# stdstu12/YUME

Measured on AMD Instinct MI355X. Metric: denoise-steps/sec (Yume-5B 720P, 33-frame latent), higher is better.
Workload: dtype bf16; 1 GPU; Yume-5B-720P random-init, 33-frame 704x1280 clip (latent 48x13x44x80, FramePack lfz=8, L=9460), ODE Euler steps of a 50-step shift-7 schedule, no CFG, one chain per GPU; num_layers=30, parallelism=dp1 (independent chains, replicated weights)

## Files before the change

yume_amd/csrc/gemm_w4.hpp:

```cpp
#pragma once
#include "gemm_core.hpp"
#include "trace.hpp"

namespace gemm_w4 {
using namespace gemm_core;

constexpr int NTHR_W4 = 256;
constexpr int OPER_BYTES = 256 * 128;
constexpr int BUF_BYTES = 2 * OPER_BYTES;
constexpr int LDS_W4 = 2 * BUF_BYTES;

#define W4_AG8(n) "a" #n "0", "a" #n "1", "a" #n "2", "a" #n "3", "a" #n "4", "a" #n "5", "a" #n "6", "a" #n "7", "a" #n "8", "a" #n "9"
#define W4_AGPRS "a0", "a1", "a2", "a3", "a4", "a5", "a6", "a7", "a8", "a9", W4_AG8(1), W4_AG8(2), W4_AG8(3), W4_AG8(4), W4_AG8(5), W4_AG8(6), \
    W4_AG8(7), W4_AG8(8), W4_AG8(9), W4_AG8(10), W4_AG8(11), W4_AG8(12), W4_AG8(13), W4_AG8(14), W4_AG8(15), W4_AG8(16), W4_AG8(17), W4_AG8(18), \
    W4_AG8(19), W4_AG8(20), W4_AG8(21), W4_AG8(22), W4_AG8(23), W4_AG8(24), "a250", "a251", "a252", "a253", "a254", "a255"

#define W4_MFMA2(T0, X0, Y0, T1, X1, Y1)                                                                                                         \
    asm volatile("v_mfma_f32_16x16x32_bf16 a[%c4:%c5], %0, %1, a[%c4:%c5]\n\tv_mfma_f32_16x16x32_bf16 a[%c6:%c7], %2, %3, a[%c6:%c7]"             \
                 ::"v"(X0), "v"(Y0), "v"(X1), "v"(Y1), "n"((T0) * 4), "n"((T0) * 4 + 3), "n"((T1) * 4), "n"((T1) * 4 + 3) : "memory", W4_AGPRS)
#define W4_MFMA2_DMA(T0, X0, Y0, T1, X1, Y1, voff, sbase, lbase, loff)                                                                            \
    asm volatile("s_add_u32 m0, %10, %11\n\tv_mfma_f32_16x16x32_bf16 a[%c4:%c5], %0, %1, a[%c4:%c5]\n\tglobal_load_lds_dwordx4 %8, %9\n\t"         \
                 "v_mfma_f32_16x16x32_bf16 a[%c6:%c7], %2, %3, a[%c6:%c7]"                                                                       \
                 ::"v"(X0), "v"(Y0), "v"(X1), "v"(Y1), "n"((T0) * 4), "n"((T0) * 4 + 3), "n"((T1) * 4), "n"((T1) * 4 + 3), "v"(voff), "s"(sbase),   \
                 "s"(lbase), "n"(loff) : "memory", "scc", W4_AGPRS)
#define W4_MFMA2_DMAB(T0, X0, Y0, T1, X1, Y1, voff, srd, soff, lbase, loff)                                                                           \
    asm volatile("s_add_u32 m0, %11, %12\n\tv_mfma_f32_16x16x32_bf16 a[%c4:%c5], %0, %1, a[%c4:%c5]\n\tbuffer_load_dwordx4 %8, %9, %10 offen lds\n\t"  \
                 "v_mfma_f32_16x16x32_bf16 a[%c6:%c7], %2, %3, a[%c6:%c7]"                                                                           \
                 ::"v"(X0), "v"(Y0), "v"(X1), "v"(Y1), "n"((T0) * 4), "n"((T0) * 4 + 3), "n"((T1) * 4), "n"((T1) * 4 + 3), "v"(voff), "s"(srd),         \
                 "s"(soff), "s"(lbase), "n"(loff) : "memory", "scc", W4_AGPRS)
#define W4_DMAB(voff, srd, soff, lbase, loff) \
    asm volatile("s_add_u32 m0, %3, %4\n\ts_nop 0\n\tbuffer_load_dwordx4 %0, %1, %2 offen lds" ::"v"(voff), "s"(srd), "s"(soff), "s"(lbase), "n"(loff) : "memory", "scc")
#define W4_DMA(voff, sbase, lbase, loff) \
    asm volatile("s_add_u32 m0, %2, %3\n\ts_nop 0\n\tglobal_load_lds_dwordx4 %0, %1" ::"v"(voff), "s"(sbase), "s"(lbase), "n"(loff) : "memory", "scc")

template <int R>
__device__ __forceinline__ f32x4 acc_tile() {
    f32x4 v;
    asm volatile("v_accvgpr_read_b32 %0, a[%c4]\n\tv_accvgpr_read_b32 %1, a[%c5]\n\tv_accvgpr_read_b32 %2, a[%c6]\n\tv_accvgpr_read_b32 %3, a[%c7]"
                 : "=v"(v[0]), "=v"(v[1]), "=v"(v[2]), "=v"(v[3]) : "n"(R * 4), "n"(R * 4 + 1), "n"(R * 4 + 2), "n"(R * 4 + 3) : W4_AGPRS);
    return v;
}
template <int R>
__device__ __forceinline__ void acc_tile_add(f32x4 d) {
    f32x4 v = acc_tile<R>();
    v += d;
    asm volatile("v_accvgpr_write_b32 a[%c4], %0\n\tv_accvgpr_write_b32 a[%c5], %1\n\tv_accvgpr_write_b32 a[%c6], %2\n\tv_accvgpr_write_b32 a[%c7], %3"
                 ::"v"(v[0]), "v"(v[1]), "v"(v[2]), "v"(v[3]), "n"(R * 4), "n"(R * 4 + 1), "n"(R * 4 + 2), "n"(R * 4 + 3) : W4_AGPRS);
}
template <int R0, int N>
__device__ __forceinline__ void acc_zero() {
    if constexpr (N > 0) {
        asm volatile("v_accvgpr_write_b32 a[%c0], 0\n\tv_accvgpr_write_b32 a[%c1], 0\n\tv_accvgpr_write_b32 a[%c2], 0\n\tv_accvgpr_write_b32 a[%c3], 0"
                     ::"n"(R0), "n"(R0 + 1), "n"(R0 + 2), "n"(R0 + 3) : W4_AGPRS);
        acc_zero<R0 + 4, N - 4>();
    }
}
template <int I0, int N, typename F>
__device__ __forceinline__ void static_for(F&& f) {
    if constexpr (N > 0) {
        f(std::integral_constant<int, I0>{});
        static_for<I0 + 1, N - 1>(f);
    }
}

struct Ctx {
    char* smem;
    bf16x8_t fa[2][8], fb[2][8];
    unsigned ra1, rb1, ra0n, rb0n;
    unsigned va[8], vb[8];
    const char* pa;
    const char* pb;
    unsigned lcur;
    i32x4 srd;
    unsigned soff, tapmask;
    unsigned mask[8];
    unsigned par[8];
    unsigned uh[2], uw[2];
};

__device__ __forceinline__ bf16x8_t w4_frag(const Ctx& c, unsigned off) { return *reinterpret_cast<const bf16x8_t*>(c.smem + off); }

#define W4_PIECE_LOFF(q) (((q) >> 3) * OPER_BYTES + ((q) & 7) * 4096)

#define W4_X(g) (SWAP ? c.fb[(g) >> 6][(g) & 7] : c.fa[(g) >> 6][((g) & 63) >> 3])
#define W4_Y(g) (SWAP ? c.fa[(g) >> 6][((g) & 63) >> 3] : c.fb[(g) >> 6][(g) & 7])
#define W4_PAIR(g) W4_MFMA2((g) & 63, W4_X(g), W4_Y(g), ((g) + 1) & 63, W4_X((g) + 1), W4_Y((g) + 1))
#define W4_PAIR_DMA(g, voff, sbase, loff) \
    W4_MFMA2_DMA((g) & 63, W4_X(g), W4_Y(g), ((g) + 1) & 63, W4_X((g) + 1), W4_Y((g) + 1), voff, sbase, c.lcur, loff)
#define W4_PAIR_DMAB(g, voff, loff) \
    W4_MFMA2_DMAB((g) & 63, W4_X(g), W4_Y(g), ((g) + 1) & 63, W4_X((g) + 1), W4_Y((g) + 1), voff, c.srd, c.soff, c.lcur, loff)

#ifndef W4_PLAN
#define W4_PLAN 1
#endif
#ifndef W4_ABLATE
#define W4_ABLATE 0
#endif
#ifndef W4_BAR_B
#define W4_BAR_B 35
#endif
#ifndef W4_BAR_A
#define W4_BAR_A 17
#endif
#ifndef W4_DMA0
#define W4_DMA0 (W4_BAR_A + 2)
#endif
constexpr int P_BAR_A = W4_BAR_A;
constexpr int P_BAR_B = W4_BAR_B;
constexpr int dma_pos(int q) { return W4_PLAN == 0 ? W4_DMA0 + q : W4_DMA0 + (q * (63 - W4_DMA0)) / 15; }
constexpr int piece_at(int pos) {
    for (int q = 0; q < 16; ++q)
        if (dma_pos(q) == pos) return q;
    return -1;
}
constexpr int pieces_before_bar_b() {
    int k = 0;
    for (int q = 0; q < 16; ++q) k += dma_pos(q) <= P_BAR_B ? 1 : 0;
    return k;
}
constexpr int P_F0_FIRST = P_BAR_B + 2;
static_assert(P_F0_FIRST + 16 <= 64 && dma_pos(15) <= 63 && 15 < P_BAR_A && dma_pos(0) > P_BAR_A, "the plan must fit the 64 slots");

template <int CONV>
__device__ __forceinline__ unsigned w4_conv_voff(const Ctx& c, int q) {
    unsigned v = c.va[q];
    if constexpr (CONV == 2) v += ((c.par[q] & 1u) ? c.uh[1] : c.uh[0]) + ((c.par[q] & 2u) ? c.uw[1] : c.uw[0]);
    return (c.mask[q] & c.tapmask) ? v : 0xffffffffu;
}

template <int g, bool DMA, bool SWAP, int CONV>
__device__ __forceinline__ void w4_gaps(Ctx& c) {
    if constexpr (g < 128) {
        {
            constexpr int k = g >> 1, pos = k;
            constexpr int q = (DMA && !(W4_ABLATE & 1)) ? piece_at(pos) : -1;
            if constexpr (q >= 0 && q < 8) {
                if constexpr (CONV != 0) W4_PAIR_DMAB(g, w4_conv_voff<CONV>(c, q & 7), W4_PIECE_LOFF(q & 15));
                else W4_PAIR_DMA(g, c.va[q & 7], c.pa, W4_PIECE_LOFF(q & 15));
            } else if constexpr (q >= 8) W4_PAIR_DMA(g, c.vb[q & 7], c.pb, W4_PIECE_LOFF(q & 15));
            else W4_PAIR(g);
            if constexpr (pos >= 0 && pos < 16 && !(W4_ABLATE & 2)) {
                if constexpr (pos < 8) c.fb[1][pos & 7] = w4_frag(c, c.rb1 + (pos & 7) * 2048);
                else c.fa[1][pos & 7] = w4_frag(c, c.ra1 + (pos & 7) * 2048);
            }
            if constexpr (k == P_BAR_A) {
                if constexpr ((W4_ABLATE & 20) == 20) asm volatile("" ::: "memory");
                else if constexpr (W4_ABLATE & 16) asm volatile("s_barrier" ::: "memory");
                else if constexpr (W4_ABLATE & 4) asm volatile("s_waitcnt lgkmcnt(0)" ::: "memory");
                else asm volatile("s_waitcnt lgkmcnt(0)\n\ts_barrier" ::: "memory");
            }
            if constexpr (k == P_BAR_B) {
                constexpr int keep = (DMA && !(W4_ABLATE & 1)) ? pieces_before_bar_b() : 0;
                if constexpr ((W4_ABLATE & 12) == 12) asm volatile("" ::: "memory");
                else if constexpr (W4_ABLATE & 8) asm volatile("s_barrier" ::: "memory");
                else if constexpr (W4_ABLATE & 4) asm volatile("s_waitcnt vmcnt(%c0)" ::"n"(keep) : "memory");
                else asm volatile("s_waitcnt vmcnt(%c0)\n\ts_barrier" ::"n"(keep) : "memory");
            }
            if constexpr (pos >= P_F0_FIRST && pos < P_F0_FIRST + 16 && !(W4_ABLATE & 2)) {
                constexpr int r = pos - P_F0_FIRST;
                if constexpr (r < 8) c.fb[0][r & 7] = w4_frag(c, c.rb0n + (r & 7) * 2048);
                else c.fa[0][r & 7] = w4_frag(c, c.ra0n + (r & 7) * 2048);
            }
            w4_gaps<g + 2, DMA, SWAP, CONV>(c);
        }
    }
}
template <int q, int CONV>
__device__ __forceinline__ void w4_stage_all(Ctx& c) {
    if constexpr (q < 16) {
        if constexpr (q < 8) {
            if constexpr (CONV != 0) W4_DMAB(w4_conv_voff<CONV>(c, q & 7), c.srd, c.soff, c.lcur, W4_PIECE_LOFF(q));
            else W4_DMA(c.va[q & 7], c.pa, c.lcur, W4_PIECE_LOFF(q));
        } else W4_DMA(c.vb[q & 7], c.pb, c.lcur, W4_PIECE_LOFF(q));
        w4_stage_all<q + 1, CONV>(c);
    }
}

template <int EPI>
__device__ __forceinline__ f32x4 w4_act(f32x4 v) {
    if (EPI == YUME_EPI_BF16_GELU) {
        const f32x2_t lo = gelu_tanh2(f32x2_t{v[0], v[1]}), hi = gelu_tanh2(f32x2_t{v[2], v[3]});
        v = f32x4{lo[0], lo[1], hi[0], hi[1]};
    }
    if (EPI == YUME_EPI_BF16_GELU_ERF) {
#pragma unroll
        for (int q = 0; q < 4; ++q) v[q] = 0.5f * v[q] * (1.0f + erff(v[q] * 0.7071067811865476f));
    }
    return v;
}

__device__ __forceinline__ void w4_store_image(char* smem, unsigned short* dst, int64_t ld, int row0, int rows_valid, int col0, int cols_valid) {
    const int lane = threadIdx.x & 63;
    const int wave = __builtin_amdgcn_readfirstlane(threadIdx.x >> 6);
    const int l31 = lane & 31, rh = lane >> 5;
    if (cols_valid == 256) {
        const unsigned lrow = (unsigned)((wave * 64 + rh) * 512), lch = (unsigned)((l31 ^ rh) << 4);
        char* o = reinterpret_cast<char*>(dst + col0 + l31 * 8) + (int64_t)(row0 + wave * 64 + rh) * ld * 2;
        const int64_t step = ld * 4;
        const int rleft = rows_valid - wave * 64 - rh;
        auto rows = [&](auto pred) {
            constexpr bool PRED = decltype(pred)::value;
#pragma unroll
            for (int g = 0; g < 4; ++g) {
                u32x4 d[8];
#pragma unroll
                for (int u = 0; u < 8; ++u) {
                    const int it = g * 8 + u;
                    d[u] = *reinterpret_cast<const u32x4*>(smem + lrow + it * 1024 + (lch ^ (unsigned)(32 * (it & 15))));
                }
#pragma unroll
                for (int u = 0; u < 8; ++u) {
                    const int it = g * 8 + u;
                    if (!PRED || 2 * it < rleft) *reinterpret_cast<u32x4*>(o + it * step) = d[u];
                }
            }
        };
        if (rows_valid == 256) rows(std::false_type{});
        else rows(std::true_type{});
        return;
    }
    unsigned short* out = dst + col0 + l31 * 8;
    const int col_left = cols_valid - l31 * 8;
#pragma unroll 2
    for (int it = 0; it < 32; ++it) {
        const int r = wave * 64 + it * 2 + rh;
        const u32x4 d = *reinterpret_cast<const u32x4*>(smem + r * 512 + (((l31 ^ r) & 31) << 4));
        if (r < rows_valid && col_left > 0) {
            unsigned short* o = out + (int64_t)(row0 + r) * ld;
            if (col_left >= 8) {
                *reinterpret_cast<u32x4*>(o) = d;
            } else {
#pragma unroll
                for (int q = 0; q < 7; ++q)
                    if (q < col_left) o[q] = (unsigned short)(d[q >> 1] >> (16 * (q & 1)));
            }
        }
    }
}

struct ImageOff { unsigned e[8], o[8]; };
__device__ __forceinline__ ImageOff w4_image_offsets(int rsel, int csel, int l15, int l4) {
    ImageOff r;
    const unsigned base = (unsigned)((rsel * 128 + l15) * 512 + (l4 & 1) * 8), ux = (unsigned)(((l4 >> 1) ^ l15) << 4);
#pragma unroll
    for (int b = 0; b < 8; ++b) {
        const unsigned ob = (unsigned)(32 * b) ^ ux;
        r.e[b] = base + 256u * (unsigned)csel + ob;
        r.o[b] = base + 256u * (unsigned)(csel ^ 1) + ob;
    }
    return r;
}

template <int EPI, bool SWAP>
__device__ __forceinline__ void w4_epilogue(const Problem& p, const Epilogue& e, int m0, int n0, char* smem) {
    const int lane = threadIdx.x & 63;
    const int wave = __builtin_amdgcn_readfirstlane(threadIdx.x >> 6);
    const int wr = wave >> 1, wc = wave & 1;
    const int l15 = lane & 15, l4 = lane >> 4;
    constexpr bool BF16_OUT = EPI == YUME_EPI_BF16 || EPI == YUME_EPI_BF16_GELU || EPI == YUME_EPI_BF16_GELU_ERF || EPI == YUME_EPI_BF16_SPLITT ||
                              EPI == EPI_BF16_ADD || EPI == EPI_BF16_TSPLIT;
    if constexpr (!SWAP) {
        float bn[8];
#pragma unroll
        for (int j = 0; j < 8; ++j) bn[j] = e.bias ? e.bias[min(n0 + wc * 128 + 16 * j + l15, p.N - 1)] : 0.f;
        const ImageOff io = w4_image_offsets(wc, wr, l15, l4);
        asm volatile("s_waitcnt lgkmcnt(0)\n\ts_barrier" ::: "memory");
        static_for<0, 64>([&](auto tt) {
            constexpr int T = decltype(tt)::value, i = T >> 3, j = T & 7;
            const f32x4 v = acc_tile<T>();
            u32x2 o;
            o[0] = pack_bf16x2(v[0] + bn[j], v[1] + bn[j]);
            o[1] = pack_bf16x2(v[2] + bn[j], v[3] + bn[j]);
            *reinterpret_cast<u32x2*>(smem + ((j & 1) ? io.o[i] : io.e[i]) + j * 8192) = o;
        });
        asm volatile("s_waitcnt lgkmcnt(0)\n\ts_barrier" ::: "memory");
        w4_store_image(smem, e.outT + (int64_t)(n0 - e.n_split) * e.ldt, e.ldt, 0, min(256, p.N - n0), m0, min(256, p.M - m0));
        return;
    } else {
        if (BF16_OUT && !p.epi_direct && (e.ldo % 8) == 0) {
            f32x4 b[8];
            if (n0 + 256 <= p.N) {
#pragma unroll
                for (int j = 0; j < 8; ++j)
                    b[j] = e.bias ? *reinterpret_cast<const f32x4*>(e.bias + n0 + wc * 128 + 16 * j + 4 * l4) : f32x4{0.f, 0.f, 0.f, 0.f};
            } else {
#pragma unroll
                for (int j = 0; j < 8; ++j) {
                    const int n = n0 + wc * 128 + 16 * j + 4 * l4;
                    b[j] = (e.bias && n + 3 < p.N) ? *reinterpret_cast<const f32x4*>(e.bias + n) : f32x4{0.f, 0.f, 0.f, 0.f};
                }
            }
            const ImageOff io = w4_image_offsets(wr, wc, l15, l4);
            asm volatile("s_waitcnt lgkmcnt(0)\n\ts_barrier" ::: "memory");
            TRACE_STAMP(3);
            static_for<0, 8>([&](auto ii) {
                constexpr int i = decltype(ii)::value;
                u32x2 a2[8];
                if constexpr (EPI == EPI_BF16_ADD) {
                    const int r = wr * 128 + 16 * i + l15;
                    const int nl = n0 + wc * 128 + 4 * l4;
                    const unsigned short* ap = e.add + (int64_t)min(m0 + r, p.M - 1) * e.ldadd + nl;
#pragma unroll
                    for (int j = 0; j < 8; ++j)
                        a2[j] = nl + 16 * j + 3 < p.N ? *reinterpret_cast<const u32x2*>(ap + 16 * j) : u32x2{0u, 0u};
                }
                static_for<0, 8>([&](auto jj) {
                    constexpr int j = decltype(jj)::value;
                    f32x4 v = w4_act<EPI>(acc_tile<i * 8 + j>() + b[j]);
                    if constexpr (EPI == EPI_BF16_ADD) {
                        v[0] += bf16_to_f32((unsigned short)(a2[j][0] & 0xffffu));
                        v[1] += bf16_to_f32((unsigned short)(a2[j][0] >> 16));
                        v[2] += bf16_to_f32((unsigned short)(a2[j][1] & 0xffffu));
                        v[3] += bf16_to_f32((unsigned short)(a2[j][1] >> 16));
                    }
                    u32x2 o;
                    o[0] = pack_bf16x2(v[0], v[1]);
                    o[1] = pack_bf16x2(v[2], v[3]);
                    *reinterpret_cast<u32x2*>(smem + ((i & 1) ? io.o[j] : io.e[j]) + i * 8192) = o;
                });
            });
            asm volatile("s_waitcnt lgkmcnt(0)\n\ts_barrier" ::: "memory");
            TRACE_STAMP(4);
            if constexpr (EPI == EPI_BF16_TSPLIT) {
                const int ch = p.N >> 1, jh = n0 >= ch ? 1 : 0, t = m0 / e.hw;
                w4_store_image(smem, reinterpret_cast<unsigned short*>(e.out), e.ldo, m0 + (t + jh) * e.hw, min(256, p.M - m0), n0 - jh * ch, 256);
            } else {
                w4_store_image(smem, reinterpret_cast<unsigned short*>(e.out), e.ldo, m0, min(256, p.M - m0), n0, min(256, p.N - n0));
            }
            return;
        }
        if (EPI == YUME_EPI_RESID && n0 + 256 <= p.N) {
            f32x4 b[8];
#pragma unroll
            for (int j = 0; j < 8; ++j)
                b[j] = e.bias ? *reinterpret_cast<const f32x4*>(e.bias + n0 + wc * 128 + 16 * j + 4 * l4) : f32x4{0.f, 0.f, 0.f, 0.f};
            const int mrow = m0 + wr * 128 + l15, ncol = n0 + wc * 128 + 4 * l4;
            const bool ragged_m = m0 + 256 > p.M;
            const int mlast = p.M - 1 - mrow;
            float* const xo = reinterpret_cast<float*>(e.out) + (int64_t)mrow * e.ldo + ncol;
            const int64_t xstep = 16 * e.ldo;
            auto xoff = [&](int i) -> int64_t { return ragged_m ? (int64_t)(min(16 * i, mlast) ) * e.ldo : i * xstep; };
            const bool gated = e.gate != nullptr;
            bool rowed = gated && e.row_idx != nullptr;
            int ridx[8];
#pragma unroll
            for (int i = 0; i < 8; ++i) ridx[i] = rowed ? e.row_idx[min(mrow + 16 * i, p.M - 1)] : 0;
            f32x4 x[2][8], g[2][8];
            auto issue_x = [&](auto ii, auto bb) {
                constexpr int i = decltype(ii)::value, bf = decltype(bb)::value;
#pragma unroll
                for (int j = 0; j < 8; ++j) x[bf][j] = *reinterpret_cast<const f32x4*>(xo + xoff(i) + 16 * j);
            };
            auto issue_g = [&](auto ii, auto bb) {
                constexpr int i = decltype(ii)::value, bf = decltype(bb)::value;
                if (rowed || (gated && i < 2)) {
                    const float* gp = e.gate + (int64_t)ridx[i] * e.gate_stride + ncol;
#pragma unroll
                    for (int j = 0; j < 8; ++j) g[bf][j] = *reinterpret_cast<const f32x4*>(gp + 16 * j);
                }
            };
            issue_x(std::integral_constant<int, 0>{}, std::integral_constant<int, 0>{});
            issue_x(std::integral_constant<int, 1>{}, std::integral_constant<int, 1>{});
            if (rowed) {
                const int r0 = __builtin_amdgcn_readfirstlane(ridx[0]);
                bool same = true;
#pragma unroll
                for (int i = 0; i < 8; ++i) same &= ridx[i] == r0;
                if (__all(same)) rowed = false;
            }
            issue_g(std::integral_constant<int, 0>{}, std::integral_constant<int, 0>{});
            issue_g(std::integral_constant<int, 1>{}, std::integral_constant<int, 1>{});
            TRACE_STAMP(3);
            static_for<0, 8>([&](auto ii) {
                constexpr int i = decltype(ii)::value, bf = i & 1;
                static_for<0, 8>([&](auto jj) {
                    constexpr int j = decltype(jj)::value;
                    const f32x4 v = acc_tile<i * 8 + j>() + b[j];
                    if (gated) x[bf][j] += v * g[bf][j];
                    else x[bf][j] += v;
                    if (!ragged_m || 16 * i <= mlast) *reinterpret_cast<f32x4*>(xo + i * xstep + 16 * j) = x[bf][j];
                });
                if constexpr (i + 2 < 8) {
                    issue_x(std::integral_constant<int, i + 2>{}, std::integral_constant<int, bf>{});
                    issue_g(std::integral_constant<int, i + 2>{}, std::integral_constant<int, bf>{});
                }
                if (i == 0) TRACE_STAMP(4);
            });
            TRACE_STAMP(5);
#ifdef YUME_TRACE
            asm volatile("s_waitcnt vmcnt(0)" ::: "memory");
            TRACE_STAMP(6);
#endif
            return;
        }
        static_for<0, 64>([&](auto tt) {
            constexpr int T = decltype(tt)::value, i = T >> 3, j = T & 7;
            const f32x4 v = acc_tile<T>();
            const int m = m0 + wr * 128 + 16 * i + l15, n = n0 + wc * 128 + 16 * j + 4 * l4;
            if (m < p.M && n < p.N) store_row4<EPI>(v, m, n, p, e);
        });
    }
}

template <bool DMA, bool SWAP>
__device__ __forceinline__ void w4_loop(Ctx& c, int t0, int t1, unsigned lbase) {
    for (int t = t0; t < t1; ++t) {
        w4_gaps<0, DMA, SWAP, 0>(c);
        if constexpr (DMA) {
            c.pa += 128;
            c.pb += 128;
        }
        c.lcur = lbase + (((t + 1) & 1) ? BUF_BYTES : 0);
        c.ra1 ^= BUF_BYTES;
        c.rb1 ^= BUF_BYTES;
        c.ra0n ^= BUF_BYTES;
        c.rb0n ^= BUF_BYTES;
    }
}

template <bool SWAP>
__device__ __forceinline__ void w4_mainloop(const Problem& p, const PlainA& al, char* smem, int m0, int n0, int kt0, int nk) {
    const int tid = threadIdx.x;
    const int lane = tid & 63;
    const int wave = __builtin_amdgcn_readfirstlane(tid >> 6);
    const int wr = wave >> 1, wc = wave & 1;
    Ctx c;
    c.smem = smem;
    const unsigned lbase = (unsigned)(uintptr_t)(__attribute__((address_space(3))) char*)smem + wave * 1024;
    c.lcur = lbase;
    c.pa = reinterpret_cast<const char*>(al.A + (int64_t)m0 * al.lda) + (int64_t)kt0 * 128;
    c.pb = reinterpret_cast<const char*>(p.W + (int64_t)n0 * p.ldw) + (int64_t)kt0 * 128;
    const unsigned lda_b = (unsigned)al.lda * 2u, ldw_b = (unsigned)p.ldw * 2u;
    {
        const int rl = 8 * wave + (lane >> 3);
        const unsigned ch = (unsigned)(((lane & 7) ^ (rl & 7)) << 4);
        const int mleft = p.M - 1 - m0, nleft = p.N - 1 - n0;
#pragma unroll
        for (int j = 0; j < 8; ++j) {
            const int r = 32 * j + rl;
            c.va[j] = (unsigned)min(r, mleft) * lda_b + ch;
            c.vb[j] = (unsigned)min(r, nleft) * ldw_b + ch;
        }
    }
    const unsigned sw0 = (unsigned)(((lane >> 4) ^ (lane & 7)) << 4), sw1 = (unsigned)(((4 | (lane >> 4)) ^ (lane & 7)) << 4);
    const unsigned rowa = wr * 16384 + (lane & 15) * 128, rowb = OPER_BYTES + wc * 16384 + (lane & 15) * 128;
    w4_stage_all<0, 0>(c);
    c.pa += 128;
    c.pb += 128;
    c.lcur = lbase + BUF_BYTES;
    w4_stage_all<0, 0>(c);
    c.pa += 128;
    c.pb += 128;
    c.lcur = lbase;
    acc_zero<0, 256>();
    asm volatile("s_waitcnt vmcnt(16)\n\ts_barrier" ::: "memory");
#pragma unroll
    for (int r = 0; r < 8; ++r) {
        c.fb[0][r] = w4_frag(c, rowb + sw0 + r * 2048);
        c.fa[0][r] = w4_frag(c, rowa + sw0 + r * 2048);
    }
    c.ra1 = rowa + sw1;
    c.rb1 = rowb + sw1;
    c.ra0n = BUF_BYTES + rowa + sw0;
    c.rb0n = BUF_BYTES + rowb + sw0;
    w4_loop<true, SWAP>(c, 0, nk - 2, lbase);
    w4_loop<false, SWAP>(c, nk - 2, nk, lbase);
    asm volatile("s_waitcnt lgkmcnt(0)\n\ts_barrier" ::: "memory");
    asm volatile("s_nop 15\n\ts_nop 15" ::: "memory");
}

constexpr int SK_SLOT_BYTES = 64 * NTHR_W4 * 16;
constexpr int SK_FLAG_STRIDE = 64;
constexpr int SK_MIN_KT = 4;
constexpr int SK_MAX_SLOTS = 256;
constexpr unsigned SK_SPIN_LIMIT = 1u << 22;

__host__ __device__ __forceinline__ int64_t sk_workspace_bytes(int slots) { return (int64_t)slots * (SK_SLOT_BYTES + SK_FLAG_STRIDE) + 64; }

template <int T0, int N>
__device__ __forceinline__ void sk_publish_tiles(const char* slot, unsigned lane_off) {
    if constexpr (N > 0) {
        const f32x4 v = acc_tile<T0>();
        asm volatile("global_store_dwordx4 %0, %1, %2 sc1\n\ts_nop 1" ::"v"(lane_off + (unsigned)(T0 * (NTHR_W4 * 16))), "v"(v), "s"(slot) : "memory");
        sk_publish_tiles<T0 + 1, N - 1>(slot, lane_off);
    }
}
template <int T0, int N>
__device__ __forceinline__ void sk_gather_tiles(const char* slot, unsigned lane_off) {
    if constexpr (N > 0) {
        f32x4 d[8];
#pragma unroll
        for (int u = 0; u < 8; ++u) d[u] = *reinterpret_cast<const f32x4*>(slot + (lane_off + (unsigned)((T0 + u) * (NTHR_W4 * 16))));
        static_for<0, 8>([&](auto uu) {
            constexpr int u = decltype(uu)::value;
            acc_tile_add<T0 + u>(d[u]);
        });
        sk_gather_tiles<T0 + 8, N - 8>(slot, lane_off);
    }
}

template <bool SWAP>
__device__ __forceinline__ void w4_finish_piece(const Problem& p, const Epilogue& e, int epi, char* smem, int m0, int n0, int slot, int t, int nslice) {
    typedef unsigned gu32;
    char* const slots = p.sk_ws;
    gu32* const flags = reinterpret_cast<gu32*>(p.sk_ws + (int64_t)SK_MAX_SLOTS * SK_SLOT_BYTES);
    unsigned lane_off = threadIdx.x * 16u;
    asm volatile("" : "+v"(lane_off));
    if (slot >= 0) {
        sk_publish_tiles<0, 64>(slots + (int64_t)slot * SK_SLOT_BYTES, lane_off);
        asm volatile("s_waitcnt vmcnt(0)" ::: "memory");
        __syncthreads();
        if (threadIdx.x == 0) __hip_atomic_store(flags + slot * (SK_FLAG_STRIDE / 4), 1u, __ATOMIC_RELAXED, __HIP_MEMORY_SCOPE_AGENT);
        return;
    }
    if (nslice > 1) {
        for (int j = 1; j < nslice; ++j) {
            const int q = (j - 1) * p.sk_tiles + t;
            if (threadIdx.x == 0) {
                gu32* f = flags + q * (SK_FLAG_STRIDE / 4);
                unsigned spins = 0;
                while (__hip_atomic_load(f, __ATOMIC_RELAXED, __HIP_MEMORY_SCOPE_AGENT) == 0u) {
                    __builtin_amdgcn_s_sleep(8);
                    if (++spins > SK_SPIN_LIMIT) {
                        __hip_atomic_store(flags + SK_MAX_SLOTS * (SK_FLAG_STRIDE / 4), 1u, __ATOMIC_RELAXED, __HIP_MEMORY_SCOPE_AGENT);
                        break;
                    }
                }
                __builtin_amdgcn_fence(__ATOMIC_ACQUIRE, "agent");
            }
            __syncthreads();
            sk_gather_tiles<0, 64>(slots + (int64_t)q * SK_SLOT_BYTES, lane_off);
            __syncthreads();
            if (threadIdx.x == 0) __hip_atomic_store(flags + q * (SK_FLAG_STRIDE / 4), 0u, __ATOMIC_RELAXED, __HIP_MEMORY_SCOPE_AGENT);
        }
        asm volatile("s_nop 15" ::: "memory");
    }
    TRACE_STAMP(1);
    if constexpr (!SWAP) {
        w4_epilogue<YUME_EPI_BF16_SPLITT, false>(p, e, m0, n0, smem);
    } else {
        switch (epi) {
#ifndef W4_EXPERIMENT
            case YUME_EPI_BF16_GELU: w4_epilogue<YUME_EPI_BF16_GELU, true>(p, e, m0, n0, smem); break;
            case YUME_EPI_BF16_GELU_ERF: w4_epilogue<YUME_EPI_BF16_GELU_ERF, true>(p, e, m0, n0, smem); break;
            case YUME_EPI_F32: w4_epilogue<YUME_EPI_F32, true>(p, e, m0, n0, smem); break;
            case YUME_EPI_RESID: w4_epilogue<YUME_EPI_RESID, true>(p, e, m0, n0, smem); break;
            case YUME_EPI_BF16_SPLITT: w4_epilogue<YUME_EPI_BF16_SPLITT, true>(p, e, m0, n0, smem); break;
#endif
            default: w4_epilogue<YUME_EPI_BF16, true>(p, e, m0, n0, smem); break;
        }
    }
}

template <int UNUSED = 0>
__global__ __launch_bounds__(NTHR_W4, 1) void gemm_w4_kernel(Problem p, PlainA al, Epilogue e, int epi) {
    __shared__ __attribute__((aligned(16))) char smem[LDS_W4];
    TRACE_STAMP(0);
    const int nk = p.K / BK;
    const int ndp = p.sk_wgs ? p.sk_dp : p.tiles_m * p.tiles_n;
    int pc0 = 0, pc1 = 1, R = 1, tile0, head_t = 0;
    bool tails = false;
    if ((int)blockIdx.x < ndp) {
        int start, count;
        xcd_chunk(ndp, blockIdx.x & 7, start, count);
        tile0 = start + (blockIdx.x >> 3);
    } else {
        const int sk = (int)blockIdx.x - ndp, per = p.sk_wgs >> 3;
        const int w = (sk & 7) * per + (sk >> 3);
        R = p.sk_tiles;
        tile0 = ndp;
        if (w < R) {
            head_t = w;
        } else {
            tails = true;
            const int ntail = (p.sk_s - 1) * R;
            pc0 = (w - R) * p.sk_q;
            pc1 = min(ntail, pc0 + p.sk_q);
            if (pc0 >= pc1) return;
        }
    }
    for (int pc = pc0; pc < pc1; ++pc) {
        int t = head_t, j = 0, k0 = 0, k1 = nk, slot = -1, nslice = 1;
        if (p.sk_wgs && (int)blockIdx.x >= ndp) {
            if (tails) {
                j = 1 + pc / R;
                t = pc - (j - 1) * R;
                k0 = p.sk_lh + (j - 1) * p.sk_lt;
                k1 = j == p.sk_s - 1 ? nk : k0 + p.sk_lt;
                slot = pc;
            } else {
                k1 = p.sk_lh;
                nslice = p.sk_s;
            }
        }
        int m0, n0;
        tile_origin(p, tile0 + t, m0, n0);
        if (epi == YUME_EPI_BF16_SPLITT && n0 >= e.n_split) {
            w4_mainloop<false>(p, al, smem, m0, n0, k0, k1 - k0);
            w4_finish_piece<false>(p, e, epi, smem, m0, n0, slot, t, nslice);
        } else {
            w4_mainloop<true>(p, al, smem, m0, n0, k0, k1 - k0);
            w4_finish_piece<true>(p, e, epi, smem, m0, n0, slot, t, nslice);
        }
        if (pc + 1 < pc1) __syncthreads();
    }
    TRACE_STAMP(2);
}

inline bool w4_applies(const Problem& p, int64_t lda, int epi) {
    if (p.K < 3 * BK) return false;
#ifdef W4_EXPERIMENT
    if (epi != YUME_EPI_BF16) return false;
#endif
    if (255ll * lda * 2 + 128 >= (1ll << 32) || 255ll * p.ldw * 2 + 128 >= (1ll << 32)) return false;
    return epi == YUME_EPI_BF16 || epi == YUME_EPI_BF16_GELU || epi == YUME_EPI_BF16_GELU_ERF || epi == YUME_EPI_F32 || epi == YUME_EPI_RESID ||
           epi == YUME_EPI_BF16_SPLITT;
}

inline void w4_sk_plan(Problem& p, void* ws, int64_t ws_bytes) {
    p.sk_dp = 0; p.sk_tiles = 0; p.sk_wgs = 0; p.sk_s = 1; p.sk_q = 1; p.sk_lh = 0; p.sk_lt = 0; p.sk_ws = nullptr;
    static const bool on = [] { const char* v = getenv("YUME_GEMM_SK"); return !v || atoi(v) != 0; }();
    static const int ncu = [] {
        int d = 0, n = 0;
        if (hipGetDevice(&d) != hipSuccess || hipDeviceGetAttribute(&n, hipDeviceAttributeMultiprocessorCount, d) != hipSuccess) n = 0;
        return n;
    }();
    if (!on || ws == nullptr || ncu < 64 || ncu > SK_MAX_SLOTS || (ncu & 7) != 0) return;
    if (ws_bytes < sk_workspace_bytes(SK_MAX_SLOTS) || ((uintptr_t)ws & 15) != 0) return;
    const int T = p.tiles_m * p.tiles_n, nk = p.K / BK;
    const int R = T % ncu;
    if (R == 0 || T < ncu) return;
    static const int min_nk = [] { const char* v = getenv("YUME_GEMM_SK_MIN_NK"); return v ? atoi(v) : 96; }();
    if (nk < min_nk) return;
    int s, q, lh, lt;
    if (2 * R > ncu) {
        s = 2;
        q = (R + (ncu - R) - 1) / (ncu - R);
        lt = nk / (q + 1);
        lh = nk - lt;
    } else {
        s = ncu / R;
        if (s > nk / SK_MIN_KT) s = nk / SK_MIN_KT;
        q = 1;
        lt = nk / s;
        lh = lt;
    }
    if (s < 2 || lt < SK_MIN_KT || lh < SK_MIN_KT || (s - 1) * R > SK_MAX_SLOTS) return;
    const int nwg = R + ((s - 1) * R + q - 1) / q;
    if (nwg > ncu) return;
    p.sk_tiles = R;
    p.sk_dp = T - R;
    p.sk_s = s; p.sk_q = q; p.sk_lh = lh; p.sk_lt = lt;
    p.sk_wgs = (nwg + 7) / 8 * 8;
    p.sk_ws = (char*)ws;
}

inline int launch_w4(int epi, const Problem& p128, const PlainA& al, const Epilogue& e, hipStream_t st, const char* what, void* ws = nullptr,
                     int64_t ws_bytes = 0) {
    Problem p = p128;
    p.tiles_m = (p.M + 255) / 256;
    p.tiles_n = (p.N + 255) / 256;
    p.group_m = g_group_m;
    { static const int d = [] { const char* v = getenv("YUME_GEMM_EPI_DIRECT"); return v ? atoi(v) : 0; }(); p.epi_direct = d; }
    w4_sk_plan(p, ws, ws_bytes);
    const unsigned grid = p.sk_wgs ? (unsigned)(p.sk_dp + p.sk_wgs) : (unsigned)(p.tiles_m * p.tiles_n);
    hipLaunchKernelGGL(gemm_w4_kernel<0>, dim3(grid), dim3(NTHR_W4), 0, st, p, al, e, epi);
    YUME_CHECK_LAUNCH(what);
    return YUME_OK;
}

}
```

yume_amd/csrc/trace.hpp:

```cpp
#pragma once
#ifdef YUME_TRACE
#include <hip/hip_runtime.h>
#define YUME_TRACE_MAX 32768
__device__ unsigned long long g_yume_trace[YUME_TRACE_MAX * 8];
__device__ __forceinline__ void trace_stamp(int slot) {
    if (threadIdx.x == 0 && blockIdx.x < YUME_TRACE_MAX) {
        g_yume_trace[blockIdx.x * 8 + slot] = __builtin_amdgcn_s_memrealtime();
        if (slot == 0)
            g_yume_trace[blockIdx.x * 8 + 7] =
                ((unsigned long long)__builtin_amdgcn_s_getreg((31 << 11) | 20) << 32) | (unsigned)__builtin_amdgcn_s_getreg((31 << 11) | 4);
    }
}
extern "C" __attribute__((visibility("default"))) int yume_debug_trace_read(void* dst, long long bytes) {
    return (int)hipMemcpyFromSymbol(dst, HIP_SYMBOL(g_yume_trace), (size_t)bytes);
}
#define TRACE_STAMP(s) trace_stamp(s)
#else
#define TRACE_STAMP(s) ((void)0)
#endif
```

Baseline: 10.26 denoise-steps/sec.

## Make W4 GEMM persistent and prefetch next tile's operands during epilogue store

When the tile count is at least twice the CU count, the non-stream-K W4 GEMM now launches one workgroup per CU, and each workgroup walks its XCD chunk of tiles with a stride. While the epilogue writes the current tile's output from LDS, the first two K-stages of the next tile are issued into the freed LDS buffers, split around the two halves of the store. This hides the per-tile prologue load latency and removes per-tile launch and scheduling cost. It adds barriers, more register and LDS-aliasing complexity, and the risk of load imbalance with fewer workgroups. Trace stamping is also reworked to record per tile.

```diff
diff --git a/yume_amd/csrc/gemm_w4.hpp b/yume_amd/csrc/gemm_w4.hpp
--- a/yume_amd/csrc/gemm_w4.hpp
+++ b/yume_amd/csrc/gemm_w4.hpp
@@ -189,19 +189,29 @@
     return v;
 }
 
-__device__ __forceinline__ void w4_store_image(char* smem, unsigned short* dst, int64_t ld, int row0, int rows_valid, int col0, int cols_valid) {
+struct W4NoStage {
+    static constexpr bool on = false;
+    static constexpr bool live = false;
+    __device__ void operator()(int) const {}
+};
+
+template <class Stage = W4NoStage>
+__device__ __forceinline__ void w4_store_image(char* smem, unsigned short* dst, int64_t ld, int row0, int rows_valid, int col0, int cols_valid,
+                                               const Stage& stage = Stage{}) {
     const int lane = threadIdx.x & 63;
     const int wave = __builtin_amdgcn_readfirstlane(threadIdx.x >> 6);
     const int l31 = lane & 31, rh = lane >> 5;
     if (cols_valid == 256) {
-        const unsigned lrow = (unsigned)((wave * 64 + rh) * 512), lch = (unsigned)((l31 ^ rh) << 4);
-        char* o = reinterpret_cast<char*>(dst + col0 + l31 * 8) + (int64_t)(row0 + wave * 64 + rh) * ld * 2;
+        const unsigned lch = (unsigned)((l31 ^ rh) << 4);
         const int64_t step = ld * 4;
-        const int rleft = rows_valid - wave * 64 - rh;
-        auto rows = [&](auto pred) {
+        auto rows = [&](auto pred, int r0, auto nit) {
             constexpr bool PRED = decltype(pred)::value;
-#pragma unroll
-            for (int g = 0; g < 4; ++g) {
+            constexpr int NIT = decltype(nit)::value;
+            const unsigned lrow = (unsigned)((r0 + rh) * 512);
+            char* o = reinterpret_cast<char*>(dst + col0 + l31 * 8) + (int64_t)(row0 + r0 + rh) * ld * 2;
+            const int rleft = rows_valid - r0 - rh;
+#pragma unroll
+            for (int g = 0; g < NIT / 8; ++g) {
                 u32x4 d[8];
 #pragma unroll
                 for (int u = 0; u < 8; ++u) {
@@ -215,8 +225,24 @@
                 }
             }
         };
-        if (rows_valid == 256) rows(std::false_type{});
-        else rows(std::true_type{});
+        auto all = [&](auto pred) {
+            if constexpr (Stage::on) {
+                rows(pred, wave * 32, std::integral_constant<int, 16>{});
+                if (stage.live) {
+                    asm volatile("s_waitcnt lgkmcnt(0)\n\ts_barrier" ::: "memory");
+                    stage(0);
+                }
+                rows(pred, 128 + wave * 32, std::integral_constant<int, 16>{});
+            } else {
+                rows(pred, wave * 64, std::integral_constant<int, 32>{});
+            }
+        };
+        if (rows_valid == 256) all(std::false_type{});
+        else all(std::true_type{});
+        if (stage.live) {
+            asm volatile("s_waitcnt lgkmcnt(0)\n\ts_barrier" ::: "memory");
+            stage(1);
+        }
         return;
     }
     unsigned short* out = dst + col0 + l31 * 8;
@@ -236,6 +262,11 @@
             }
         }
     }
+    if (stage.live) {
+        asm volatile("s_waitcnt lgkmcnt(0)\n\ts_barrier" ::: "memory");
+        stage(0);
+        stage(1);
+    }
 }
 
 struct ImageOff { unsigned e[8], o[8]; };
@@ -251,8 +282,9 @@
     return r;
 }
 
-template <int EPI, bool SWAP>
-__device__ __forceinline__ void w4_epilogue(const Problem& p, const Epilogue& e, int m0, int n0, char* smem) {
+constexpr int W4_UNSTAGED = 0, W4_STAGED_IMAGE = 1, W4_STAGED_FIRST = 2;
+template <int EPI, bool SWAP, class Stage = W4NoStage>
+__device__ __forceinline__ int w4_epilogue(const Problem& p, const Epilogue& e, int m0, int n0, char* smem, const Stage& stage = Stage{}) {
     const int lane = threadIdx.x & 63;
     const int wave = __builtin_amdgcn_readfirstlane(threadIdx.x >> 6);
     const int wr = wave >> 1, wc = wave & 1;
@@ -274,8 +306,8 @@
             *reinterpret_cast<u32x2*>(smem + ((j & 1) ? io.o[i] : io.e[i]) + j * 8192) = o;
         });
         asm volatile("s_waitcnt lgkmcnt(0)\n\ts_barrier" ::: "memory");
-        w4_store_image(smem, e.outT + (int64_t)(n0 - e.n_split) * e.ldt, e.ldt, 0, min(256, p.N - n0), m0, min(256, p.M - m0));
-        return;
+        w4_store_image(smem, e.outT + (int64_t)(n0 - e.n_split) * e.ldt, e.ldt, 0, min(256, p.N - n0), m0, min(256, p.M - m0), stage);
+        return stage.live ? W4_STAGED_IMAGE : W4_UNSTAGED;
     } else {
         if (BF16_OUT && !p.epi_direct && (e.ldo % 8) == 0) {
             f32x4 b[8];
@@ -323,11 +355,15 @@
             TRACE_STAMP(4);
             if constexpr (EPI == EPI_BF16_TSPLIT) {
                 const int ch = p.N >> 1, jh = n0 >= ch ? 1 : 0, t = m0 / e.hw;
-                w4_store_image(smem, reinterpret_cast<unsigned short*>(e.out), e.ldo, m0 + (t + jh) * e.hw, min(256, p.M - m0), n0 - jh * ch, 256);
+                w4_store_image(smem, reinterpret_cast<unsigned short*>(e.out), e.ldo, m0 + (t + jh) * e.hw, min(256, p.M - m0), n0 - jh * ch, 256, stage);
             } else {
-                w4_store_image(smem, reinterpret_cast<unsigned short*>(e.out), e.ldo, m0, min(256, p.M - m0), n0, min(256, p.N - n0));
-            }
-            return;
+                w4_store_image(smem, reinterpret_cast<unsigned short*>(e.out), e.ldo, m0, min(256, p.M - m0), n0, min(256, p.N - n0), stage);
+            }
+            return stage.live ? W4_STAGED_IMAGE : W4_UNSTAGED;
+        }
+        if (stage.live) {
+            stage(0);
+            stage(1);
         }
         if (EPI == YUME_EPI_RESID && n0 + 256 <= p.N) {
             f32x4 b[8];
@@ -387,11 +423,7 @@
                 if (i == 0) TRACE_STAMP(4);
             });
             TRACE_STAMP(5);
-#ifdef YUME_TRACE
-            asm volatile("s_waitcnt vmcnt(0)" ::: "memory");
-            TRACE_STAMP(6);
-#endif
-            return;
+            return stage.live ? W4_STAGED_FIRST : W4_UNSTAGED;
         }
         static_for<0, 64>([&](auto tt) {
             constexpr int T = decltype(tt)::value, i = T >> 3, j = T & 7;
@@ -399,6 +431,7 @@
             const int m = m0 + wr * 128 + 16 * i + l15, n = n0 + wc * 128 + 16 * j + 4 * l4;
             if (m < p.M && n < p.N) store_row4<EPI>(v, m, n, p, e);
         });
+        return stage.live ? W4_STAGED_FIRST : W4_UNSTAGED;
     }
 }
 
@@ -418,42 +451,69 @@
     }
 }
 
-template <bool SWAP>
-__device__ __forceinline__ void w4_mainloop(const Problem& p, const PlainA& al, char* smem, int m0, int n0, int kt0, int nk) {
-    const int tid = threadIdx.x;
-    const int lane = tid & 63;
-    const int wave = __builtin_amdgcn_readfirstlane(tid >> 6);
-    const int wr = wave >> 1, wc = wave & 1;
-    Ctx c;
+__device__ __forceinline__ unsigned w4_sources(Ctx& c, const Problem& p, const PlainA& al, char* smem, int m0, int n0, int kt0) {
+    const int lane = threadIdx.x & 63;
+    const int wave = __builtin_amdgcn_readfirstlane(threadIdx.x >> 6);
     c.smem = smem;
     const unsigned lbase = (unsigned)(uintptr_t)(__attribute__((address_space(3))) char*)smem + wave * 1024;
     c.lcur = lbase;
     c.pa = reinterpret_cast<const char*>(al.A + (int64_t)m0 * al.lda) + (int64_t)kt0 * 128;
     c.pb = reinterpret_cast<const char*>(p.W + (int64_t)n0 * p.ldw) + (int64_t)kt0 * 128;
     const unsigned lda_b = (unsigned)al.lda * 2u, ldw_b = (unsigned)p.ldw * 2u;
-    {
-        const int rl = 8 * wave + (lane >> 3);
-        const unsigned ch = (unsigned)(((lane & 7) ^ (rl & 7)) << 4);
-        const int mleft = p.M - 1 - m0, nleft = p.N - 1 - n0;
-#pragma unroll
-        for (int j = 0; j < 8; ++j) {
-            const int r = 32 * j + rl;
-            c.va[j] = (unsigned)min(r, mleft) * lda_b + ch;
-            c.vb[j] = (unsigned)min(r, nleft) * ldw_b + ch;
-        }
-    }
+    const int rl = 8 * wave + (lane >> 3);
+    const unsigned ch = (unsigned)(((lane & 7) ^ (rl & 7)) << 4);
+    const int mleft = p.M - 1 - m0, nleft = p.N - 1 - n0;
+#pragma unroll
+    for (int j = 0; j < 8; ++j) {
+        const int r = 32 * j + rl;
+        c.va[j] = (unsigned)min(r, mleft) * lda_b + ch;
+        c.vb[j] = (unsigned)min(r, nleft) * ldw_b + ch;
+    }
+    return lbase;
+}
+
+struct W4Stage {
+    static constexpr bool on = true;
+    const Problem* p;
+    const PlainA* al;
+    char* smem;
+    int m0, n0;
+    bool live;
+    __device__ __forceinline__ void operator()(int k) const {
+        Ctx c;
+        const unsigned lbase = w4_sources(c, *p, *al, smem, m0, n0, k);
+        c.lcur = lbase + (k ? BUF_BYTES : 0);
+        w4_stage_all<0, 0>(c);
+    }
+};
+
+template <bool SWAP>
+__device__ __forceinline__ void w4_mainloop(const Problem& p, const PlainA& al, char* smem, int m0, int n0, int kt0, int nk, int staged) {
+    const int tid = threadIdx.x;
+    const int lane = tid & 63;
+    const int wave = __builtin_amdgcn_readfirstlane(tid >> 6);
+    const int wr = wave >> 1, wc = wave & 1;
+    Ctx c;
+    const unsigned lbase = w4_sources(c, p, al, smem, m0, n0, kt0);
     const unsigned sw0 = (unsigned)(((lane >> 4) ^ (lane & 7)) << 4), sw1 = (unsigned)(((4 | (lane >> 4)) ^ (lane & 7)) << 4);
     const unsigned rowa = wr * 16384 + (lane & 15) * 128, rowb = OPER_BYTES + wc * 16384 + (lane & 15) * 128;
-    w4_stage_all<0, 0>(c);
-    c.pa += 128;
-    c.pb += 128;
-    c.lcur = lbase + BUF_BYTES;
-    w4_stage_all<0, 0>(c);
-    c.pa += 128;
-    c.pb += 128;
-    c.lcur = lbase;
+    if (staged == W4_UNSTAGED) {
+        w4_stage_all<0, 0>(c);
+        c.pa += 128;
+        c.pb += 128;
+        c.lcur = lbase + BUF_BYTES;
+        w4_stage_all<0, 0>(c);
+        c.pa += 128;
+        c.pb += 128;
+        c.lcur = lbase;
+    } else {
+        c.pa += 256;
+        c.pb += 256;
+    }
     acc_zero<0, 256>();
-    asm volatile("s_waitcnt vmcnt(16)\n\ts_barrier" ::: "memory");
+    if (staged == W4_STAGED_FIRST) asm volatile("s_waitcnt vmcnt(0)\n\ts_barrier" ::: "memory");
+    else asm volatile("s_waitcnt vmcnt(16)\n\ts_barrier" ::: "memory");
+    TRACE_STAMP(6);
 #pragma unroll
     for (int r = 0; r < 8; ++r) {
         c.fb[0][r] = w4_frag(c, rowb + sw0 + r * 2048);
@@ -500,7 +560,8 @@
 }
 
 template <bool SWAP>
-__device__ __forceinline__ void w4_finish_piece(const Problem& p, const Epilogue& e, int epi, char* smem, int m0, int n0, int slot, int t, int nslice) {
+__device__ __forceinline__ int w4_finish_piece(const Problem& p, const Epilogue& e, int epi, char* smem, int m0, int n0, int slot, int t, int nslice,
+                                               const W4Stage& nx) {
     typedef unsigned gu32;
     char* const slots = p.sk_ws;
     gu32* const flags = reinterpret_cast<gu32*>(p.sk_ws + (int64_t)SK_MAX_SLOTS * SK_SLOT_BYTES);
@@ -511,7 +572,7 @@
         asm volatile("s_waitcnt vmcnt(0)" ::: "memory");
         __syncthreads();
         if (threadIdx.x == 0) __hip_atomic_store(flags + slot * (SK_FLAG_STRIDE / 4), 1u, __ATOMIC_RELAXED, __HIP_MEMORY_SCOPE_AGENT);
-        return;
+        return W4_UNSTAGED;
     }
     if (nslice > 1) {
         for (int j = 1; j < nslice; ++j) {
@@ -537,17 +598,17 @@
     }
     TRACE_STAMP(1);
     if constexpr (!SWAP) {
-        w4_epilogue<YUME_EPI_BF16_SPLITT, false>(p, e, m0, n0, smem);
+        return w4_epilogue<YUME_EPI_BF16_SPLITT, false>(p, e, m0, n0, smem, nx);
     } else {
         switch (epi) {
 #ifndef W4_EXPERIMENT
-            case YUME_EPI_BF16_GELU: w4_epilogue<YUME_EPI_BF16_GELU, true>(p, e, m0, n0, smem); break;
-            case YUME_EPI_BF16_GELU_ERF: w4_epilogue<YUME_EPI_BF16_GELU_ERF, true>(p, e, m0, n0, smem); break;
-            case YUME_EPI_F32: w4_epilogue<YUME_EPI_F32, true>(p, e, m0, n0, smem); break;
-            case YUME_EPI_RESID: w4_epilogue<YUME_EPI_RESID, true>(p, e, m0, n0, smem); break;
-            case YUME_EPI_BF16_SPLITT: w4_epilogue<YUME_EPI_BF16_SPLITT, true>(p, e, m0, n0, smem); break;
+            case YUME_EPI_BF16_GELU: return w4_epilogue<YUME_EPI_BF16_GELU, true>(p, e, m0, n0, smem, nx);
+            case YUME_EPI_BF16_GELU_ERF: return w4_epilogue<YUME_EPI_BF16_GELU_ERF, true>(p, e, m0, n0, smem, nx);
+            case YUME_EPI_F32: return w4_epilogue<YUME_EPI_F32, true>(p, e, m0, n0, smem, nx);
+            case YUME_EPI_RESID: return w4_epilogue<YUME_EPI_RESID, true>(p, e, m0, n0, smem, nx);
+            case YUME_EPI_BF16_SPLITT: return w4_epilogue<YUME_EPI_BF16_SPLITT, true>(p, e, m0, n0, smem, nx);
 #endif
-            default: w4_epilogue<YUME_EPI_BF16, true>(p, e, m0, n0, smem); break;
+            default: return w4_epilogue<YUME_EPI_BF16, true>(p, e, m0, n0, smem, nx);
         }
     }
 }
@@ -555,12 +616,20 @@
 template <int UNUSED = 0>
 __global__ __launch_bounds__(NTHR_W4, 1) void gemm_w4_kernel(Problem p, PlainA al, Epilogue e, int epi) {
     __shared__ __attribute__((aligned(16))) char smem[LDS_W4];
-    TRACE_STAMP(0);
     const int nk = p.K / BK;
     const int ndp = p.sk_wgs ? p.sk_dp : p.tiles_m * p.tiles_n;
-    int pc0 = 0, pc1 = 1, R = 1, tile0, head_t = 0;
-    bool tails = false;
-    if ((int)blockIdx.x < ndp) {
+    int pc0 = 0, pc1 = 1, step = 1, R = 1, tile0, head_t = 0;
+    bool tails = false, walk = false;
+    if (p.sk_wgs) TRACE_STAMP(0);
+    if (!p.sk_wgs && (int)gridDim.x < ndp) {
+        int start, count;
+        xcd_chunk(ndp, blockIdx.x & 7, start, count);
+        tile0 = start;
+        pc0 = blockIdx.x >> 3;
+        pc1 = count;
+        step = gridDim.x >> 3;
+        walk = true;
+    } else if ((int)blockIdx.x < ndp) {
         int start, count;
         xcd_chunk(ndp, blockIdx.x & 7, start, count);
         tile0 = start + (blockIdx.x >> 3);
@@ -579,8 +648,9 @@
             if (pc0 >= pc1) return;
         }
     }
-    for (int pc = pc0; pc < pc1; ++pc) {
-        int t = head_t, j = 0, k0 = 0, k1 = nk, slot = -1, nslice = 1;
+    int staged = W4_UNSTAGED;
+    for (int pc = pc0; pc < pc1; pc += step) {
+        int t = walk ? pc : head_t, j = 0, k0 = 0, k1 = nk, slot = -1, nslice = 1;
         if (p.sk_wgs && (int)blockIdx.x >= ndp) {
             if (tails) {
                 j = 1 + pc / R;
@@ -595,16 +665,20 @@
         }
         int m0, n0;
         tile_origin(p, tile0 + t, m0, n0);
+        if (!p.sk_wgs) TRACE_START(tile0 + t);
+        W4Stage nx{&p, &al, smem, 0, 0, walk && pc + step < pc1};
+        if (nx.live) tile_origin(p, tile0 + pc + step, nx.m0, nx.n0);
         if (epi == YUME_EPI_BF16_SPLITT && n0 >= e.n_split) {
-            w4_mainloop<false>(p, al, smem, m0, n0, k0, k1 - k0);
-            w4_finish_piece<false>(p, e, epi, smem, m0, n0, slot, t, nslice);
+            w4_mainloop<false>(p, al, smem, m0, n0, k0, k1 - k0, staged);
+            staged = w4_finish_piece<false>(p, e, epi, smem, m0, n0, slot, t, nslice, nx);
         } else {
-            w4_mainloop<true>(p, al, smem, m0, n0, k0, k1 - k0);
-            w4_finish_piece<true>(p, e, epi, smem, m0, n0, slot, t, nslice);
-        }
-        if (pc + 1 < pc1) __syncthreads();
-    }
-    TRACE_STAMP(2);
+            w4_mainloop<true>(p, al, smem, m0, n0, k0, k1 - k0, staged);
+            staged = w4_finish_piece<true>(p, e, epi, smem, m0, n0, slot, t, nslice, nx);
+        }
+        if (!p.sk_wgs) TRACE_STAMP(2);
+        if (staged == W4_UNSTAGED && pc + step < pc1) __syncthreads();
+    }
+    if (p.sk_wgs) TRACE_STAMP(2);
 }
 
 inline bool w4_applies(const Problem& p, int64_t lda, int epi) {
@@ -655,6 +729,17 @@
     p.sk_ws = (char*)ws;
 }
 
+inline unsigned w4_dp_grid(int T) {
+    static const bool on = [] { const char* v = getenv("YUME_GEMM_PERSIST"); return !v || atoi(v) != 0; }();
+    static const int ncu = [] {
+        int d = 0, n = 0;
+        if (hipGetDevice(&d) != hipSuccess || hipDeviceGetAttribute(&n, hipDeviceAttributeMultiprocessorCount, d) != hipSuccess) n = 0;
+        return n;
+    }();
+    if (!on || ncu < 8 || (ncu & 7) != 0 || T < 2 * ncu) return (unsigned)T;
+    return (unsigned)ncu;
+}
+
 inline int launch_w4(int epi, const Problem& p128, const PlainA& al, const Epilogue& e, hipStream_t st, const char* what, void* ws = nullptr,
                      int64_t ws_bytes = 0) {
     Problem p = p128;
@@ -663,7 +748,7 @@
     p.group_m = g_group_m;
     { static const int d = [] { const char* v = getenv("YUME_GEMM_EPI_DIRECT"); return v ? atoi(v) : 0; }(); p.epi_direct = d; }
     w4_sk_plan(p, ws, ws_bytes);
-    const unsigned grid = p.sk_wgs ? (unsigned)(p.sk_dp + p.sk_wgs) : (unsigned)(p.tiles_m * p.tiles_n);
+    const unsigned grid = p.sk_wgs ? (unsigned)(p.sk_dp + p.sk_wgs) : w4_dp_grid(p.tiles_m * p.tiles_n);
     hipLaunchKernelGGL(gemm_w4_kernel<0>, dim3(grid), dim3(NTHR_W4), 0, st, p, al, e, epi);
     YUME_CHECK_LAUNCH(what);
     return YUME_OK;
diff --git a/yume_amd/csrc/trace.hpp b/yume_amd/csrc/trace.hpp
--- a/yume_amd/csrc/trace.hpp
+++ b/yume_amd/csrc/trace.hpp
@@ -3,18 +3,26 @@
 #include <hip/hip_runtime.h>
 #define YUME_TRACE_MAX 32768
 __device__ unsigned long long g_yume_trace[YUME_TRACE_MAX * 8];
+__shared__ unsigned g_yume_trace_rec;
 __device__ __forceinline__ void trace_stamp(int slot) {
-    if (threadIdx.x == 0 && blockIdx.x < YUME_TRACE_MAX) {
-        g_yume_trace[blockIdx.x * 8 + slot] = __builtin_amdgcn_s_memrealtime();
-        if (slot == 0)
-            g_yume_trace[blockIdx.x * 8 + 7] =
+    if (threadIdx.x == 0 && g_yume_trace_rec < YUME_TRACE_MAX) g_yume_trace[g_yume_trace_rec * 8 + slot] = __builtin_amdgcn_s_memrealtime();
+}
+__device__ __forceinline__ void trace_start(unsigned rec) {
+    if (threadIdx.x == 0) {
+        g_yume_trace_rec = rec;
+        if (rec < YUME_TRACE_MAX) {
+            g_yume_trace[rec * 8] = __builtin_amdgcn_s_memrealtime();
+            g_yume_trace[rec * 8 + 7] =
                 ((unsigned long long)__builtin_amdgcn_s_getreg((31 << 11) | 20) << 32) | (unsigned)__builtin_amdgcn_s_getreg((31 << 11) | 4);
+        }
     }
 }
 extern "C" __attribute__((visibility("default"))) int yume_debug_trace_read(void* dst, long long bytes) {
     return (int)hipMemcpyFromSymbol(dst, HIP_SYMBOL(g_yume_trace), (size_t)bytes);
 }
-#define TRACE_STAMP(s) trace_stamp(s)
+#define TRACE_STAMP(s) ((s) == 0 ? trace_start(blockIdx.x) : trace_stamp(s))
+#define TRACE_START(r) trace_start(r)
 #else
 #define TRACE_STAMP(s) ((void)0)
+#define TRACE_START(r) ((void)0)
 #endif
```

New measurement: 10.29 denoise-steps/sec, median of 6. No clear change (+0.3%).
